# jim-ec/constraint_solver

Measured on AMD Instinct MI355X. Metric: body·substeps/sec at 262k rigid bodies, 20 substeps/frame; 1/2/4/8 GPU, higher is better.
Workload: dtype f64

## Files before the change

constraint_solver_amd/csrc/xpbd_pairs.h:

```cpp
#pragma once

#include <cstdint>
#include <hip/hip_runtime_api.h>

#include "xpbd_kernels.h"

namespace xpbd {

struct ShapeDesc {
    uint32_t vert0, n_verts;
    uint32_t face0, n_faces;
    uint32_t edge0, n_edges;
    uint32_t dir0, n_dirs;
};

struct PolytopeTables {
    const double *verts;
    const double *planes;
    const double *centroids;
    const ShapeDesc *desc;
    const uint32_t *face_start;
    const uint32_t *face_verts;
    const uint32_t *edges;
    const double *radii;
    const double *edge_dirs;
    const uint32_t *edge_dir_id;
    uint32_t n_shapes;
    uint32_t total_verts;
    uint32_t max_verts, max_faces, max_face_verts;
    const uint8_t *shape_class;
    uint32_t two_classes;
    uint32_t small_max_face_verts;
};

constexpr uint32_t kMaxManifoldPoints = 8;
constexpr uint32_t kMaxFaceVerts = 8;
constexpr double kEdgeBias = 1e-6;

struct Manifold {
    uint32_t n_points;
    uint32_t feature;
    uint32_t index_a, index_b;
    double separation;
    double p_ref[kMaxManifoldPoints][3];
    double p_inc[kMaxManifoldPoints][3];
};

struct alignas(256) ContactManifold {
    double plane[4];
    double point[kMaxManifoldPoints][3];
};
static_assert(sizeof(ContactManifold) == 256, "plane + four points = the first 128-byte line");
constexpr uint32_t kPairCodeFeatureShift = 4;
constexpr uint32_t kSurvivorCounters = 4;

struct EdgeQuery {
    double separation;
    uint32_t edge_a, edge_b;
};
hipError_t launch_edge_axes_reference(const BodyArrays &b, const PolytopeTables &t, const double *frames, const uint32_t *pairs,
                                      uint32_t n_pairs, EdgeQuery *out, hipStream_t stream);


struct SatScratch {
    uint32_t *counters;
    uint32_t *survivors;
    uint32_t calls;
    uint16_t *axis_cache;
    bool cache_edge_axes;
};

hipError_t launch_sat_pairs(const BodyArrays &b, const PolytopeTables &t, const double *frames, const uint32_t *pairs,
                            uint32_t n_pairs, Manifold *out, hipStream_t stream);
hipError_t launch_pair_pretest(const BodyArrays &b, const PolytopeTables &t, const double *frames, const uint32_t *pairs,
                               uint32_t n_pairs, uint8_t *codes, SatScratch &list, uint32_t **count, uint32_t **next_count,
                               hipStream_t stream, bool use_axis_cache = false, const double *gjk_axis_cache = nullptr);
hipError_t launch_sat_contacts(const BodyArrays &b, const PolytopeTables &t, const double *frames, const uint32_t *pairs,
                               uint32_t n_pairs, ContactManifold *out, uint8_t *codes, SatScratch *list,
                               hipStream_t stream, bool dense = false);

}
```

constraint_solver_amd/csrc/xpbd_pairs.hip:

```cpp
#include <cfloat>
#include <cstdlib>

#include <type_traits>

#include "xpbd_clip.hpp"
#include "xpbd_device.hpp"
#include "xpbd_pairs.h"

namespace xpbd {
namespace {

constexpr uint32_t kMaxV = XPBD_MAX_SHAPE_VERTS;
#ifndef XPBD_SAT_MIN_WAVES_PER_SIMD
#define XPBD_SAT_MIN_WAVES_PER_SIMD 4
#endif
#ifndef XPBD_SAT_BOX_LANES
#define XPBD_SAT_BOX_LANES 8
#endif
#ifndef XPBD_SAT_DENSE_BOX_LANES
#define XPBD_SAT_DENSE_BOX_LANES 4
#endif
#ifndef XPBD_SAT_SMALL_LANES
#define XPBD_SAT_SMALL_LANES 16
#endif
#ifndef XPBD_SAT_LS_LANES
#define XPBD_SAT_LS_LANES 16
#endif
#ifndef XPBD_SAT_MID_LANES
#define XPBD_SAT_MID_LANES 32
#endif
#ifndef XPBD_SAT_TIMING_STOP
#define XPBD_SAT_TIMING_STOP 0
#endif
#ifndef XPBD_SAT_EDGE_CACHE_GAP
#define XPBD_SAT_EDGE_CACHE_GAP 1.0e-5
#endif
constexpr uint32_t kNone = 0xFFFFFFFFu;
constexpr uint32_t kAxisCacheEdge = 0x8000u;
constexpr uint32_t kWidePairCount = 32768;

template <uint32_t V, uint32_t P, uint32_t PW>
struct PairLds {
    static constexpr uint32_t kVerts = V;
    static_assert(kMaxFaceVerts <= V, "the reference face reuses vertex rows");
    static constexpr uint32_t kScratchRows = P > V ? P : V;
    static constexpr uint32_t kBaseDwords = 2 * (2 * V * 3 + 2 * kScratchRows * 3);
    static constexpr uint32_t pad_dwords()
    {
        if (PW == 1)
            return 0;
        uint32_t best = 64;
        for (uint32_t odd = 1; odd < 2 * PW; odd += 2) {
            const uint32_t pad = (odd * (64 / PW) + 64 - kBaseDwords % 64) % 64;
            best = pad < best ? pad : best;
        }
        return best;
    }
    static constexpr uint32_t kPadDwords = pad_dwords();
    double world[2][V][3];
    union {
        double local[2][V][3];
        double poly[2][P][3];
    };
    uint32_t pad[kPadDwords ? kPadDwords : 2];
};

__device__ __forceinline__ bool finite3(Vec3 v)
{
    return fabs(v.x) <= DBL_MAX && fabs(v.y) <= DBL_MAX && fabs(v.z) <= DBL_MAX;
}

__device__ __forceinline__ Vec3 support_last_max(const double (*verts)[3], uint32_t n, Vec3 dir)
{
    Vec3 best = ld3(verts, 0);
    long long best_key = total_key(dot(best, dir));
    for (uint32_t k = 1; k < n; ++k) {
        const Vec3 x = ld3(verts, k);
        const long long key = total_key(dot(x, dir));
        if (best_key <= key) {
            best_key = key;
            best = x;
        }
    }
    return best;
}

__device__ __forceinline__ double clamp01(double x) { return x < 0.0 ? 0.0 : (x > 1.0 ? 1.0 : x); }

template <uint32_t L, class Lds, class M>
__device__ __forceinline__ void sat_pair(Lds &s, const BodyArrays &b, const PolytopeTables &t, const double *__restrict__ frames,
                                         const uint32_t *__restrict__ pairs, uint32_t p, M *__restrict__ out, uint32_t lane,
                                         uint16_t *__restrict__ axis_cache = nullptr, uint8_t *__restrict__ codes = nullptr, bool cache_edge_axes = false)
{
    constexpr uint32_t H = L / 2;
    constexpr uint32_t P = (Lds::kVerts <= 8 && L <= 8) ? 8 : 16;
    const uint32_t ia = pairs[2 * (size_t)p], ib = pairs[2 * (size_t)p + 1];
    const Frame fa = load_record_p1(frames, ia), fb = load_record_p1(frames, ib);
    const Frame fa_inv = inverse(fa), fb_inv = inverse(fb);
    const uint32_t sa = b.shape_id[ia], sb = b.shape_id[ib];
    const ShapeDesc da = t.desc[sa], db = t.desc[sb];

    M *m = out + p;
    auto answer = [&](uint32_t n_points, uint32_t feature, uint32_t index_a, uint32_t index_b, double separation) {
        if (codes)
            codes[p] = (uint8_t)(n_points | (feature << kPairCodeFeatureShift));
        set_header(*m, n_points, feature, index_a, index_b, separation);
    };
    auto no_contact = [&]() {
        if (codes)
            codes[p] = 0;
        else
            set_header(*m, 0, 0, 0, 0, 0.0);
    };
    if (da.n_verts == 0 || db.n_verts == 0 || da.n_faces == 0 || db.n_faces == 0) {
        if (lane == 0)
            no_contact();
        return;
    }

    const uint32_t half = lane / H, k = lane % H;
    {
        const ShapeDesc dm = half ? db : da;
        for (uint32_t vtx = k; vtx < dm.n_verts; vtx += H) {
            const double *v = t.verts + 3 * (size_t)(dm.vert0 + vtx);
            const Vec3 w = (half ? fb : fa) * Vec3{v[0], v[1], v[2]};
            st3(s.world[half], vtx, w);
            st3(s.local[half], vtx, (half ? fa_inv : fb_inv) * w);
        }
    }
    __syncthreads();

    double fdist = -DBL_MAX;
    uint32_t fidx = kNone;
    {
        const ShapeDesc dm = half ? db : da;
        const uint32_t n_other = half ? da.n_verts : db.n_verts;
        for (uint32_t f = k; f < dm.n_faces; f += H) {
            const double *pl = t.planes + 4 * (size_t)(dm.face0 + f);
            const Vec3 n{pl[0], pl[1], pl[2]};
            const Vec3 sup = support_last_max(s.local[half ^ 1u], n_other, -n);
            const double dist = dot(n, sup) - pl[3];
            if (dist > fdist) {
                fdist = dist;
                fidx = f;
            }
        }
    }
    reduce_max_first(fdist, fidx, H);
    const double fdist_other = partner(fdist, H);
    const uint32_t fidx_other = partner(fidx, H);
    const double qa = half ? fdist_other : fdist, qb = half ? fdist : fdist_other;
    const uint32_t face_a = half ? fidx_other : fidx, face_b = half ? fidx : fidx_other;
    if (qa >= 0.0 || qb >= 0.0 || face_a == kNone || face_b == kNone) {
        if (lane == 0) {
            no_contact();
            if (axis_cache)
                axis_cache[p] = (uint16_t)(qa >= 0.0 ? 1u + 2u * face_a : (qb >= 0.0 ? 2u + 2u * face_b : 0u));
        }
        return;
    }
    if (axis_cache && lane == 0)
        axis_cache[p] = 0;
#if XPBD_SAT_TIMING_STOP == 1
    if (lane == 0)
        no_contact();
    return;
#endif

    double ebest = -DBL_MAX;
    uint32_t eq = kNone;
    const double *cca = t.centroids + 3 * (size_t)sa, *ccb = t.centroids + 3 * (size_t)sb;
    const Vec3 a_to_b = fb * Vec3{ccb[0], ccb[1], ccb[2]} - fa * Vec3{cca[0], cca[1], cca[2]};
    const bool dirs_staged = da.n_dirs <= Lds::kVerts && db.n_dirs <= Lds::kVerts;
    __syncthreads();
    if (dirs_staged) {
        for (uint32_t d = lane; d < da.n_dirs + db.n_dirs; d += L) {
            const bool of_b = d >= da.n_dirs;
            const uint32_t kd = of_b ? d - da.n_dirs : d;
            const double *dd = t.edge_dirs + 3 * (size_t)((of_b ? db.dir0 : da.dir0) + kd);
            st3(s.local[of_b ? 1 : 0], kd, (of_b ? fb : fa).rotation * Vec3{dd[0], dd[1], dd[2]});
        }
        __syncthreads();
    }
    auto edge_axis = [&](uint32_t i, uint32_t j, Vec3 &axis) -> bool {
        Vec3 n;
        if (dirs_staged) {
            n = normalized(cross(ld3(s.local[0], i), ld3(s.local[1], j)));
        } else {
            const double *da_ = t.edge_dirs + 3 * (size_t)(da.dir0 + i), *db_ = t.edge_dirs + 3 * (size_t)(db.dir0 + j);
            n = normalized(cross(fa.rotation * Vec3{da_[0], da_[1], da_[2]}, fb.rotation * Vec3{db_[0], db_[1], db_[2]}));
        }
        if (!finite3(n))
            return false;
        if (dot(n, a_to_b) < 0.0)
            n = -n;
        axis = n;
        return true;
    };
    {
        const uint32_t total = da.n_dirs * db.n_dirs;
        for (uint32_t q = lane; q < total; q += L) {
            const uint32_t i = q / db.n_dirs, j = q - i * db.n_dirs;
            Vec3 axis;
            if (!edge_axis(i, j, axis))
                continue;
            double reach_a = dot(ld3(s.world[0], 0), axis), reach_b = dot(ld3(s.world[1], 0), axis);
            for (uint32_t v = 1; v < da.n_verts; ++v) {
                const double rr = dot(ld3(s.world[0], v), axis);
                if (rr > reach_a)
                    reach_a = rr;
            }
            for (uint32_t v = 1; v < db.n_verts; ++v) {
                const double rr = dot(ld3(s.world[1], v), axis);
                if (rr < reach_b)
                    reach_b = rr;
            }
            const double dist = reach_b - reach_a;
            if (dist > ebest) {
                ebest = dist;
                eq = q;
            }
        }
    }
    reduce_max_first(ebest, eq, L);
    if (ebest >= 0.0) {
        if (lane == 0) {
            no_contact();
            if (axis_cache && cache_edge_axes && ebest > XPBD_SAT_EDGE_CACHE_GAP)
                axis_cache[p] = (uint16_t)(kAxisCacheEdge | eq);
        }
        return;
    }

#if XPBD_SAT_TIMING_STOP == 2
    if (lane == 0)
        no_contact();
    return;
#endif
    const double face_best = qa > qb ? qa : qb;
    const bool use_edges = eq != kNone && ebest > face_best + kEdgeBias;

    if (use_edges) {
        const uint32_t di = eq / db.n_dirs, dj = eq - di * db.n_dirs;
        Vec3 axis;
        (void)edge_axis(di, dj, axis);
        double sa_best = -DBL_MAX, sb_best = DBL_MAX;
        uint32_t edge_i = kNone, edge_j = kNone;
        for (uint32_t e = lane; e < da.n_edges; e += L) {
            if (t.edge_dir_id[da.edge0 + e] != di)
                continue;
            const uint32_t *ev = t.edges + 2 * (size_t)(da.edge0 + e);
            const double sp = dot(ld3(s.world[0], ev[0]), axis) + dot(ld3(s.world[0], ev[1]), axis);
            if (sp > sa_best) {
                sa_best = sp;
                edge_i = e;
            }
        }
        for (uint32_t e = lane; e < db.n_edges; e += L) {
            if (t.edge_dir_id[db.edge0 + e] != dj)
                continue;
            const uint32_t *ev = t.edges + 2 * (size_t)(db.edge0 + e);
            const double sp = dot(ld3(s.world[1], ev[0]), axis) + dot(ld3(s.world[1], ev[1]), axis);
            if (sp < sb_best) {
                sb_best = sp;
                edge_j = e;
            }
        }
        reduce_max_first(sa_best, edge_i, L);
        reduce_min_first(sb_best, edge_j, L);
        if (edge_i == kNone)
            edge_i = 0;
        if (edge_j == kNone)
            edge_j = 0;
        if (lane == 0) {
            const uint32_t i = edge_i, j = edge_j;
            const uint32_t *ea = t.edges + 2 * (size_t)(da.edge0 + i), *eb = t.edges + 2 * (size_t)(db.edge0 + j);
            const Vec3 a0 = ld3(s.world[0], ea[0]), a1 = ld3(s.world[0], ea[1]);
            const Vec3 b0 = ld3(s.world[1], eb[0]), b1 = ld3(s.world[1], eb[1]);
            const Vec3 d1 = a1 - a0, d2 = b1 - b0, r = a0 - b0;
            const double a = dot(d1, d1), e = dot(d2, d2), f = dot(d2, r), c = dot(d1, r), bb = dot(d1, d2);
            const double denom = a * e - bb * bb;
            double sp = clamp01((bb * f - c * e) / denom);
            double tp = (bb * sp + f) / e;
            if (tp < 0.0) {
                tp = 0.0;
                sp = clamp01(-c / a);
            } else if (tp > 1.0) {
                tp = 1.0;
                sp = clamp01((bb - c) / a);
            }
            const Vec3 pa = a0 + d1 * sp, pb = b0 + d2 * tp;
            answer(1, 2, i, j, ebest);
            set_single_contact(*m, pb, pa);
        }
        return;
    }

    const uint32_t r = (qa == face_best) ? 0u : 1u;
    const uint32_t ref_face = r ? face_b : face_a;
    const Frame fr = r ? fb : fa, fi = r ? fa : fb;
    const ShapeDesc dr = r ? db : da, di = r ? da : db;
    uint32_t iface;
    const uint32_t n_out = face_contact_group<L, P>(t, dr, di, fr, fi, ref_face, s.world[r], s.world[r ^ 1u], s.poly[0], s.poly[1],
                                                    s.world[r ^ 1u], m, lane, iface);
    if (lane != 0)
        return;
    answer(n_out, r, r ? iface : face_a, r ? face_b : iface, face_best);
}

__device__ __forceinline__ bool tight_spheres_overlap(const BodyArrays &b, const PolytopeTables &t, const double *__restrict__ frames,
                                                      const uint32_t *__restrict__ pairs, uint32_t p)
{
    const uint32_t ia = pairs[2 * (size_t)p], ib = pairs[2 * (size_t)p + 1];
    const uint32_t sa = b.shape_id[ia], sb = b.shape_id[ib];
    const double *ca = t.centroids + 3 * (size_t)sa, *cb = t.centroids + 3 * (size_t)sb;
    const Vec3 between = load_record_p1(frames, ib) * Vec3{cb[0], cb[1], cb[2]} - load_record_p1(frames, ia) * Vec3{ca[0], ca[1], ca[2]};
    const double reach = t.radii[sa] + t.radii[sb];
    return dot(between, between) < reach * reach;
}

template <uint32_t L, uint32_t V>
struct SatLds {
    static constexpr uint32_t PW = 64 / L;
    static constexpr uint32_t P = (V <= 8 && L <= 8) ? 8 : 16;
    static_assert(V == 8 || V == 16 || V == kMaxV, "vertex capacity per body");
    using Record = PairLds<V, P, PW>;
    static_assert(sizeof(Record) % 8 == 0, "pair records must stay 8-byte aligned");
};

template <uint32_t L, uint32_t V, bool PRETEST, class M>
__global__ void __launch_bounds__(64, XPBD_SAT_MIN_WAVES_PER_SIMD) k_sat_pairs(BodyArrays b, PolytopeTables t,
                                                                               const double *__restrict__ frames,
                                                                               const uint32_t *__restrict__ pairs, uint32_t n_pairs,
                                                                               M *__restrict__ out, uint8_t *__restrict__ codes)
{
    using Lds = typename SatLds<L, V>::Record;
    __shared__ Lds s_all[SatLds<L, V>::PW];
    const uint32_t group = threadIdx.x / L, lane = threadIdx.x % L;
    const uint32_t p = blockIdx.x * SatLds<L, V>::PW + group;
    if (p >= n_pairs)
        return;
    if (PRETEST && !tight_spheres_overlap(b, t, frames, pairs, p)) {
        if (lane == 0)
            codes[p] = 0;
        return;
    }
    sat_pair<L>(s_all[group], b, t, frames, pairs, p, out, lane, nullptr, codes);
}

constexpr uint32_t kPretestBlock = 1024;

__device__ __forceinline__ bool cached_direction_separates(const BodyArrays &b, const PolytopeTables &t, const double *__restrict__ frames,
                                                           const uint32_t *__restrict__ pairs, uint32_t p, Vec3 d)
{
    const uint32_t ia = pairs[2 * (size_t)p], ib = pairs[2 * (size_t)p + 1];
    const Frame fa = load_record_p1(frames, ia), fb = load_record_p1(frames, ib);
    const ShapeDesc da = t.desc[b.shape_id[ia]], db = t.desc[b.shape_id[ib]];
    if (da.n_verts == 0 || db.n_verts == 0)
        return false;
    auto support = [&](const ShapeDesc &ds, Vec3 dir) {
        Vec3 best{0.0, 0.0, 0.0};
        long long best_key = 0;
        for (uint32_t k = 0; k < ds.n_verts; ++k) {
            const double *v = t.verts + 3 * (size_t)(ds.vert0 + k);
            const Vec3 x{v[0], v[1], v[2]};
            const long long key = total_key(dot(x, dir));
            if (k == 0 || best_key <= key) {
                best_key = key;
                best = x;
            }
        }
        return best;
    };
    const Vec3 a = fa * support(da, conjugate(fa.rotation) * d), bb = fb * support(db, conjugate(fb.rotation) * (-d));
    return !(dot(a - bb, d) > 0.0);
}

__device__ __forceinline__ bool cached_face_separates(const BodyArrays &b, const PolytopeTables &t, const double *__restrict__ frames,
                                                      const uint32_t *__restrict__ pairs, uint32_t p, uint32_t code)
{
    const uint32_t owner = (code - 1u) & 1u, face = (code - 1u) >> 1;
    const uint32_t ia = pairs[2 * (size_t)p], ib = pairs[2 * (size_t)p + 1];
    const Frame fa = load_record_p1(frames, ia), fb = load_record_p1(frames, ib);
    const ShapeDesc da = t.desc[b.shape_id[ia]], db = t.desc[b.shape_id[ib]];
    const ShapeDesc dx = owner ? db : da, dy = owner ? da : db;
    if (face >= dx.n_faces || dy.n_verts == 0)
        return false;
    const Frame fy = owner ? fa : fb, fx_inv = inverse(owner ? fb : fa);
    const double *pl = t.planes + 4 * (size_t)(dx.face0 + face);
    const Vec3 n{pl[0], pl[1], pl[2]}, dir = -n;
    Vec3 best{0.0, 0.0, 0.0};
    long long best_key = 0;
    for (uint32_t k = 0; k < dy.n_verts; ++k) {
        const double *v = t.verts + 3 * (size_t)(dy.vert0 + k);
        const Vec3 w = fy * Vec3{v[0], v[1], v[2]};
        const Vec3 local = fx_inv * w;
        const long long key = total_key(dot(local, dir));
        if (k == 0 || best_key <= key) {
            best_key = key;
            best = local;
        }
    }
    return dot(n, best) - pl[3] >= 0.0;
}

__device__ __forceinline__ bool cached_edge_axis_separates(const BodyArrays &b, const PolytopeTables &t, const double *__restrict__ frames,
                                                           const uint32_t *__restrict__ pairs, uint32_t p, uint32_t q)
{
    const uint32_t ia = pairs[2 * (size_t)p], ib = pairs[2 * (size_t)p + 1];
    const Frame fa = load_record_p1(frames, ia), fb = load_record_p1(frames, ib);
    const uint32_t sa = b.shape_id[ia], sb = b.shape_id[ib];
    const ShapeDesc da = t.desc[sa], db = t.desc[sb];
    if (da.n_verts == 0 || db.n_verts == 0 || db.n_dirs == 0)
        return false;
    const uint32_t i = q / db.n_dirs, j = q - i * db.n_dirs;
    if (i >= da.n_dirs)
        return false;
    const double *da_ = t.edge_dirs + 3 * (size_t)(da.dir0 + i), *db_ = t.edge_dirs + 3 * (size_t)(db.dir0 + j);
    Vec3 n = normalized(cross(fa.rotation * Vec3{da_[0], da_[1], da_[2]}, fb.rotation * Vec3{db_[0], db_[1], db_[2]}));
    if (!finite3(n))
        return false;
    const double *cca = t.centroids + 3 * (size_t)sa, *ccb = t.centroids + 3 * (size_t)sb;
    const Vec3 a_to_b = fb * Vec3{ccb[0], ccb[1], ccb[2]} - fa * Vec3{cca[0], cca[1], cca[2]};
    if (dot(n, a_to_b) < 0.0)
        n = -n;
    double reach_a = 0.0, reach_b = 0.0;
    for (uint32_t v = 0; v < da.n_verts; ++v) {
        const double *x = t.verts + 3 * (size_t)(da.vert0 + v);
        const double rr = dot(fa * Vec3{x[0], x[1], x[2]}, n);
        if (v == 0 || rr > reach_a)
            reach_a = rr;
    }
    for (uint32_t v = 0; v < db.n_verts; ++v) {
        const double *x = t.verts + 3 * (size_t)(db.vert0 + v);
        const double rr = dot(fb * Vec3{x[0], x[1], x[2]}, n);
        if (v == 0 || rr < reach_b)
            reach_b = rr;
    }
    return reach_b - reach_a >= 0.0;
}

template <bool CLASSES>
__global__ void __launch_bounds__(kPretestBlock) k_pair_pretest(BodyArrays b, PolytopeTables t, const double *__restrict__ frames,
                                                                const uint32_t *__restrict__ pairs, uint32_t n_pairs,
                                                                uint8_t *__restrict__ codes, uint32_t *__restrict__ survivor_count,
                                                                uint32_t *__restrict__ survivors, const uint16_t *__restrict__ axis_cache,
                                                                const double *__restrict__ gjk_axis_cache)
{
    constexpr uint32_t NC = CLASSES ? 3 : 1;
    constexpr uint32_t NP = 3, NW = kPretestBlock / 64;
    __shared__ uint32_t wave_base[NC][NP][NW];
    __shared__ uint32_t list_base[NC];
    const uint32_t p = blockIdx.x * kPretestBlock + threadIdx.x, lane = threadIdx.x & 63u, wave = threadIdx.x >> 6;
    bool keep = false;
    uint32_t cls = 0, path = 0;
    if (p < n_pairs) {
        const uint32_t last = codes[p];
        path = last == 0 ? 0u : ((last >> kPairCodeFeatureShift) == 2u ? 2u : 1u);
        keep = tight_spheres_overlap(b, t, frames, pairs, p);
        if (keep && axis_cache) {
            const uint32_t code = axis_cache[p];
            if (code & kAxisCacheEdge ? cached_edge_axis_separates(b, t, frames, pairs, p, code & (kAxisCacheEdge - 1u))
                                      : (code && cached_face_separates(b, t, frames, pairs, p, code)))
                keep = false;
        }
        if (keep && gjk_axis_cache) {
            const double *c = gjk_axis_cache + 3 * (size_t)p;
            const Vec3 d{c[0], c[1], c[2]};
            if (dot(d, d) > 0.0 && cached_direction_separates(b, t, frames, pairs, p, d))
                keep = false;
        }
        if (!keep)
            codes[p] = 0;
        else if (CLASSES) {
            const uint32_t ca = t.shape_class[b.shape_id[pairs[2 * (size_t)p]]], cb = t.shape_class[b.shape_id[pairs[2 * (size_t)p + 1]]];
            cls = ca + cb;
        }
    }
    unsigned long long mine = 0;
#pragma unroll
    for (uint32_t c = 0; c < NC; ++c)
#pragma unroll
        for (uint32_t q = 0; q < NP; ++q) {
            const unsigned long long mask = __ballot(keep && cls == c && path == q);
            if (lane == 0)
                wave_base[c][q][wave] = (uint32_t)__popcll(mask);
            if (cls == c && path == q)
                mine = mask;
        }
    __syncthreads();
    if (threadIdx.x < NC) {
        const uint32_t c = threadIdx.x;
        uint32_t run = 0;
        for (uint32_t q = 0; q < NP; ++q)
            for (uint32_t w = 0; w < NW; ++w) {
                const uint32_t n = wave_base[c][q][w];
                wave_base[c][q][w] = run;
                run += n;
            }
        list_base[c] = run ? atomicAdd(survivor_count + c, run) : 0u;
    }
    __syncthreads();
    if (keep) {
        const uint32_t at = list_base[cls] + wave_base[cls][path][wave] + (uint32_t)__popcll(mine & ((1ull << lane) - 1ull));
        survivors[cls == 0 ? at : (cls == 1 ? n_pairs - 1u - at : n_pairs + at)] = p;
    }
}

template <uint32_t L, uint32_t V>
__global__ void __launch_bounds__(64, XPBD_SAT_MIN_WAVES_PER_SIMD) k_sat_survivors(BodyArrays b, PolytopeTables t,
                                                                                   const double *__restrict__ frames,
                                                                                   const uint32_t *__restrict__ pairs,
                                                                                   const uint32_t *__restrict__ survivor_count,
                                                                                   uint32_t *__restrict__ next_survivor_counts,
                                                                                   const uint32_t *__restrict__ survivors, uint32_t back_n,
                                                                                   ContactManifold *__restrict__ out, uint16_t *__restrict__ axis_cache,
                                                                                   uint8_t *__restrict__ codes, bool cache_edge_axes)
{
    using Lds = typename SatLds<L, V>::Record;
    __shared__ Lds s_all[SatLds<L, V>::PW];
    const uint32_t group = threadIdx.x / L, lane = threadIdx.x % L;
    const uint32_t k = blockIdx.x * SatLds<L, V>::PW + group;
    const uint32_t n = *survivor_count;
    if (blockIdx.x == 0 && threadIdx.x < kSurvivorCounters)
        next_survivor_counts[threadIdx.x] = 0;
    if (k >= n)
        return;
    sat_pair<L>(s_all[group], b, t, frames, pairs, survivors[back_n ? back_n - 1u - k : k], out, lane, axis_cache, codes, cache_edge_axes);
}

struct EdgeLds {
    double world[2][kMaxV][3];
};

__device__ __forceinline__ Vec3 support_last_max_position(const double (*verts)[3], uint32_t n, Vec3 dir)
{
    return support_last_max(verts, n, dir);
}

__global__ void __launch_bounds__(64) k_edge_axes_reference(BodyArrays b, PolytopeTables t, const double *__restrict__ frames,
                                                            const uint32_t *__restrict__ pairs, uint32_t n_pairs, EdgeQuery *__restrict__ out)
{
    __shared__ EdgeLds s;
    const uint32_t p = blockIdx.x, lane = threadIdx.x;
    if (p >= n_pairs)
        return;
    const uint32_t ia = pairs[2 * (size_t)p], ib = pairs[2 * (size_t)p + 1];
    const Frame fa = load_record_p1(frames, ia), fb = load_record_p1(frames, ib);
    const uint32_t sa = b.shape_id[ia], sb = b.shape_id[ib];
    const ShapeDesc da = t.desc[sa], db = t.desc[sb];
    for (uint32_t v = lane; v < da.n_verts + db.n_verts; v += 64) {
        const bool of_b = v >= da.n_verts;
        const uint32_t k = of_b ? v - da.n_verts : v;
        const double *x = t.verts + 3 * (size_t)((of_b ? db.vert0 : da.vert0) + k);
        st3(s.world[of_b ? 1 : 0], k, (of_b ? fb : fa) * Vec3{x[0], x[1], x[2]});
    }
    __syncthreads();
    const double *cca = t.centroids + 3 * (size_t)sa;
    const Vec3 centroid_a = fa * Vec3{cca[0], cca[1], cca[2]};
    double best = -DBL_MAX;
    uint32_t best_q = kNone;
    const uint32_t total = da.n_edges * db.n_edges;
    for (uint32_t q = lane; q < total; q += 64) {
        const uint32_t ie = q / db.n_edges, je = q - ie * db.n_edges;
        const uint32_t *ea = t.edges + 2 * (size_t)(da.edge0 + ie), *eb = t.edges + 2 * (size_t)(db.edge0 + je);
        const Vec3 foot = ld3(s.world[0], ea[0]);
        const Vec3 e0 = ld3(s.world[0], ea[1]) - foot;
        const Vec3 e1 = ld3(s.world[1], eb[1]) - ld3(s.world[1], eb[0]);
        Vec3 axis = normalized(cross(e0, e1));
        if (dot(axis, foot - centroid_a) < 0.0)
            axis = -axis;
        if (da.n_verts == 0 || db.n_verts == 0)
            continue;
        if (dot(support_last_max_position(s.world[0], da.n_verts, axis), axis) > dot(foot, axis))
            continue;
        const Plane plane = plane_from_point_normal(foot, axis);
        const double dist = distance(plane, support_last_max_position(s.world[1], db.n_verts, -axis));
        if (dist > best) {
            best = dist;
            best_q = q;
        }
    }
    reduce_max_first(best, best_q, 64);
    if (lane == 0) {
        out[p].separation = best;
        out[p].edge_a = best_q == kNone ? kNone : best_q / db.n_edges;
        out[p].edge_b = best_q == kNone ? kNone : best_q % db.n_edges;
    }
}

}

namespace {
uint32_t wide_pair_count()
{
    const char *e = std::getenv("XPBD_SAT_WIDE_PAIRS");
    return e ? (uint32_t)std::strtoul(e, nullptr, 10) : kWidePairCount;
}

template <class Launch>
void for_shape_maxima(uint32_t max_verts, uint32_t max_faces, uint32_t max_face_verts, uint32_t n_pairs, bool dense, Launch launch)
{
    const uint32_t wide = wide_pair_count();
    if (max_verts <= 8 && max_faces <= 8 && max_face_verts <= 4 && dense && n_pairs >= 2 * (size_t)wide)
        launch(std::integral_constant<uint32_t, XPBD_SAT_DENSE_BOX_LANES>{}, std::integral_constant<uint32_t, 8>{});
    else if (max_verts <= 8 && max_faces <= 8 && max_face_verts <= 4 && n_pairs >= wide)
        launch(std::integral_constant<uint32_t, XPBD_SAT_BOX_LANES>{}, std::integral_constant<uint32_t, 8>{});
    else if (max_verts <= 8 && max_faces <= 8)
        launch(std::integral_constant<uint32_t, XPBD_SAT_SMALL_LANES>{}, std::integral_constant<uint32_t, 8>{});
    else if (max_verts <= 16)
        launch(std::integral_constant<uint32_t, XPBD_SAT_MID_LANES>{}, std::integral_constant<uint32_t, 16>{});
    else
        launch(std::integral_constant<uint32_t, 64>{}, std::integral_constant<uint32_t, kMaxV>{});
}

template <class Launch>
void for_shape_class(const PolytopeTables &t, uint32_t n_pairs, bool dense, Launch launch)
{
    for_shape_maxima(t.max_verts, t.max_faces, t.max_face_verts, n_pairs, dense, launch);
}
}

hipError_t launch_sat_pairs(const BodyArrays &b, const PolytopeTables &t, const double *frames, const uint32_t *pairs,
                            uint32_t n_pairs, Manifold *out, hipStream_t stream)
{
    if (n_pairs)
        for_shape_class(t, n_pairs, false, [&](auto lanes, auto verts) {
            constexpr uint32_t L = decltype(lanes)::value, V = decltype(verts)::value;
            hipLaunchKernelGGL((k_sat_pairs<L, V, false, Manifold>), dim3((n_pairs + 64 / L - 1) / (64 / L)), dim3(64), 0, stream, b, t,
                               frames, pairs, n_pairs, out, nullptr);
        });
    return hipGetLastError();
}

hipError_t launch_edge_axes_reference(const BodyArrays &b, const PolytopeTables &t, const double *frames, const uint32_t *pairs,
                                      uint32_t n_pairs, EdgeQuery *out, hipStream_t stream)
{
    if (n_pairs)
        hipLaunchKernelGGL(k_edge_axes_reference, dim3(n_pairs), dim3(64), 0, stream, b, t, frames, pairs, n_pairs, out);
    return hipGetLastError();
}

hipError_t launch_pair_pretest(const BodyArrays &b, const PolytopeTables &t, const double *frames, const uint32_t *pairs,
                               uint32_t n_pairs, uint8_t *codes, SatScratch &list, uint32_t **count, uint32_t **next_count,
                               hipStream_t stream, bool use_axis_cache, const double *gjk_axis_cache)
{
    *count = list.counters + kSurvivorCounters * (list.calls & 1u);
    *next_count = list.counters + kSurvivorCounters * ((list.calls + 1u) & 1u);
    ++list.calls;
    hipLaunchKernelGGL(k_pair_pretest<false>, dim3((n_pairs + kPretestBlock - 1) / kPretestBlock), dim3(kPretestBlock), 0, stream, b, t, frames,
                       pairs, n_pairs, codes, *count, list.survivors, use_axis_cache ? list.axis_cache : nullptr, gjk_axis_cache);
    return hipGetLastError();
}

hipError_t launch_sat_contacts(const BodyArrays &b, const PolytopeTables &t, const double *frames, const uint32_t *pairs,
                               uint32_t n_pairs, ContactManifold *out, uint8_t *codes, SatScratch *list, hipStream_t stream, bool dense)
{
    if (n_pairs == 0)
        return hipSuccess;
    if (list && t.two_classes) {
        uint32_t *count = list->counters + kSurvivorCounters * (list->calls & 1u);
        uint32_t *next = list->counters + kSurvivorCounters * ((list->calls + 1u) & 1u);
        ++list->calls;
        hipLaunchKernelGGL(k_pair_pretest<true>, dim3((n_pairs + kPretestBlock - 1) / kPretestBlock), dim3(kPretestBlock), 0, stream, b, t,
                           frames, pairs, n_pairs, codes, count, list->survivors, list->axis_cache, nullptr);
        for_shape_maxima(8, 8, t.small_max_face_verts, n_pairs, dense, [&](auto lanes, auto verts) {
            constexpr uint32_t L = decltype(lanes)::value, V = decltype(verts)::value;
            hipLaunchKernelGGL((k_sat_survivors<L, V>), dim3((n_pairs + 64 / L - 1) / (64 / L)), dim3(64), 0, stream, b, t, frames, pairs, count,
                               next, list->survivors, 0u, out, list->axis_cache, codes, list->cache_edge_axes);
        });
        if (t.max_verts <= 16)
            hipLaunchKernelGGL((k_sat_survivors<XPBD_SAT_LS_LANES, 16>), dim3((n_pairs + 64 / XPBD_SAT_LS_LANES - 1) / (64 / XPBD_SAT_LS_LANES)), dim3(64), 0,
                               stream, b, t, frames, pairs, count + 1, next, list->survivors, n_pairs, out, list->axis_cache, codes, list->cache_edge_axes);
        else
            hipLaunchKernelGGL((k_sat_survivors<32, kMaxV>), dim3((n_pairs + 1) / 2), dim3(64), 0, stream, b, t, frames, pairs, count + 1, next,
                               list->survivors, n_pairs, out, list->axis_cache, codes, list->cache_edge_axes);
        for_shape_class(t, n_pairs, dense, [&](auto lanes, auto verts) {
            constexpr uint32_t L = decltype(lanes)::value, V = decltype(verts)::value;
            hipLaunchKernelGGL((k_sat_survivors<L, V>), dim3((n_pairs + 64 / L - 1) / (64 / L)), dim3(64), 0, stream, b, t, frames, pairs,
                               count + 2, next, list->survivors + n_pairs, 0u, out, list->axis_cache, codes, list->cache_edge_axes);
        });
        return hipGetLastError();
    }
    for_shape_class(t, n_pairs, dense, [&](auto lanes, auto verts) {
        constexpr uint32_t L = decltype(lanes)::value, V = decltype(verts)::value;
        const dim3 grid((n_pairs + 64 / L - 1) / (64 / L));
        if (list) {
            uint32_t *count = nullptr, *next = nullptr;
            (void)launch_pair_pretest(b, t, frames, pairs, n_pairs, codes, *list, &count, &next, stream, true);
            hipLaunchKernelGGL((k_sat_survivors<L, V>), grid, dim3(64), 0, stream, b, t, frames, pairs, count, next, list->survivors, 0u, out,
                               list->axis_cache, codes, list->cache_edge_axes);
        } else {
            hipLaunchKernelGGL((k_sat_pairs<L, V, true, ContactManifold>), grid, dim3(64), 0, stream, b, t, frames, pairs, n_pairs, out, codes);
        }
    });
    return hipGetLastError();
}

}
```

constraint_solver_amd/csrc/xpbd_world.hpp:

```cpp
#pragma once

#include <cstdint>
#include <limits>
#include <utility>
#include <vector>

#include <hip/hip_runtime_api.h>

#include "xpbd_internal.h"
#include "xpbd_kernels.h"
#include "xpbd_contacts.h"
#include "xpbd_gjk.h"
#include "xpbd_islands.h"
#include "xpbd_joint_state.h"
#include "xpbd_kinematic.h"
#include "xpbd_pairs.h"
#include "xpbd_population_remap.hpp"
#include "xpbd_query.h"
#include "xpbd_report.h"
#include "xpbd_sleep.h"

struct xpbd_world;

#pragma GCC visibility push(hidden)

using xpbd::DeviceBuffer;
using xpbd::set_error;

constexpr uint32_t kMaxBodies = 0xFFFFFF00u;
template <class T> constexpr T at_least_one(T n) { return n ? n : 1; }
inline uint32_t stride_for(uint32_t n_bodies) { return (at_least_one(n_bodies) + 255u) / 256u * 256u; }
inline uint32_t next_pow2(uint32_t v)
{
    uint32_t p = 1;
    while (p < v)
        p <<= 1;
    return p;
}

struct JointTables {
    xpbd::JointSet set;
    std::vector<xpbd_joint_limit> slide_limits;
    struct Csr {
        uint32_t n = 0;
        DeviceBuffer joints, off, list;
    } csr;
    struct Limits {
        uint32_t n_limits = 0;
        DeviceBuffer limits, limit_off;
    } limits;
    struct Extras {
        uint32_t n_extra_joints = 0;
        DeviceBuffer sums, joints, slots, off, items;
        DeviceBuffer joint_slot, drive_item;
        std::vector<uint32_t> drive_item_host;
        bool targets_on_device = false;
    } extras;

    void fill(xpbd::ContactBuffers &c) const
    {
        c.joints = csr.joints.as<xpbd::Joint>();
        c.joint_off = csr.off.as<uint32_t>();
        c.joint_list = csr.list.as<uint32_t>();
        c.limits = limits.limits.as<xpbd::JointLimit>();
        c.limit_off = limits.limit_off.as<uint32_t>();
        c.joint_extra = extras.sums.as<double>();
        c.extra_joints = extras.joints.as<uint32_t>();
        c.extra_slots = extras.slots.as<uint32_t>();
        c.extra_off = extras.off.as<uint32_t>();
        c.extra_items = extras.items.as<xpbd::JointExtraItem>();
        c.n_extra_joints = extras.n_extra_joints;
    }
    xpbd::JointStateTables state_tables() const
    {
        return xpbd::JointStateTables{csr.joints.as<xpbd::Joint>(), csr.n, limits.limits.as<xpbd::JointLimit>(), limits.limit_off.as<uint32_t>(),
                                      extras.joint_slot.as<uint32_t>(), extras.off.as<uint32_t>(), extras.items.as<xpbd::JointExtraItem>()};
    }
    xpbd::DriveTable drive_table() const
    {
        return xpbd::DriveTable{extras.items.as<xpbd::JointExtraItem>(), extras.drive_item.as<uint32_t>(), (uint32_t)extras.drive_item_host.size()};
    }
    void clear() { *this = JointTables{}; }
};

struct KinematicBodies {
    std::vector<xpbd_kinematic> list;
    DeviceBuffer table;
    bool targets_on_device = false;

    bool any() const { return !list.empty(); }
    xpbd::KinematicTable view() const { return xpbd::KinematicTable{table.as<xpbd_kinematic>(), (uint32_t)list.size()}; }
    void clear() { *this = KinematicBodies{}; }
};

struct Broadphase {
    DeviceBuffer centers, radius, cell, key, maxr, grid_partials, bucket_start, bucket_cursor, items, items_unsorted, slot_sphere,
        slot_cell, slot_filter, slot_inert, nbr_off, pair_first, upper_start, nbr, nbr_pair, pairs, manifolds, pair_codes, scan;
    uint32_t table_size = 0, n_entries = 0, n_pairs = 0;
    bool have_neighbours = false;
    struct Totals {
        uint32_t entries, pairs;
        unsigned long long stats[2];
    };
    Totals *totals = nullptr;
    hipEvent_t event = nullptr;
    bool pending = false;

    Broadphase() = default;
    Broadphase(const Broadphase &) = delete;
    Broadphase &operator=(const Broadphase &) = delete;
    ~Broadphase() { release_host(); }
    void release_host() noexcept
    {
        if (totals)
            (void)hipHostFree(totals);
        if (event)
            (void)hipEventDestroy(event);
        totals = nullptr;
        event = nullptr;
    }
    void fill(xpbd::ContactBuffers &c) const
    {
        c.centers = centers.as<double>();
        c.radius = radius.as<double>();
        c.cell = cell.as<int32_t>();
        c.key = key.as<uint32_t>();
        c.grid = maxr.as<xpbd::GridInfo>();
        c.grid_partials = grid_partials.as<double>();
        c.bucket_start = bucket_start.as<uint32_t>();
        c.bucket_cursor = bucket_cursor.as<uint32_t>();
        c.items = items.as<uint32_t>();
        c.items_unsorted = items_unsorted.as<uint32_t>();
        c.table_size = table_size;
        c.slot_sphere = slot_sphere.as<double>();
        c.slot_cell = slot_cell.as<int32_t>();
        c.nbr_off = nbr_off.as<uint32_t>();
        c.pair_first = pair_first.as<uint32_t>();
        c.upper_start = upper_start.as<uint32_t>();
        c.nbr = nbr.as<uint32_t>();
        c.nbr_pair = nbr_pair.as<uint32_t>();
        c.pairs = pairs.as<uint32_t>();
        c.manifolds = manifolds.as<xpbd::ContactManifold>();
        c.pair_codes = pair_codes.as<uint8_t>();
        c.scan_scratch = scan.as<uint32_t>();
    }
};

struct NarrowphaseSchedule {
    DeviceBuffer stats;
    DeviceBuffer sat_counters, sat_survivors, sat_axis_cache, gjk_axis_cache;
    xpbd::SatScratch sat_scratch{nullptr, nullptr, 0, nullptr, true};
    bool sat_two_pass = false;
    uint32_t sat_schedule = XPBD_SAT_SCHEDULE_AUTO;
    unsigned long long stats_touching_seen = 0, stats_pair_substeps = 0, stats_pair_substeps_seen = 0;
    DeviceBuffer gjk_counters, gjk_pairs_scratch;
    xpbd::GjkScratch gjk_scratch{nullptr, nullptr, 0, nullptr, nullptr};

    void choose(unsigned long long touching_now, uint32_t two_classes);
    int ensure_gjk_scratch(uint32_t n_pairs, hipStream_t stream);
};

struct ContactReport {
    bool on = false;
    bool frame = false;
    bool keys_ready = false;
    bool ready = false;
    bool prev_valid = false;
    uint32_t substeps = 0, cur = 0;
    uint32_t counts[4] = {0, 0, 0, 0};
    uint32_t *host = nullptr;
    DeviceBuffer touch, flag, sel, npts, keys[2], scan, ev_flag, pairs, points, events;
    const uint8_t *map_owned = nullptr;
    const uint32_t *map_ids = nullptr;

    ContactReport() = default;
    ContactReport(const ContactReport &) = delete;
    ContactReport &operator=(const ContactReport &) = delete;
    ~ContactReport() { release_host(); }
    void release_host() noexcept
    {
        if (host)
            (void)hipHostFree(host);
        host = nullptr;
    }

    void reset()
    {
        frame = keys_ready = ready = prev_valid = false;
        substeps = 0;
    }
    void release_buffers()
    {
        for (DeviceBuffer *b : {&touch, &flag, &sel, &npts, &keys[0], &keys[1], &scan, &ev_flag, &pairs, &points, &events})
            b->release();
    }
    xpbd::ReportFrame frame_of(const Broadphase &bp) const
    {
        return xpbd::ReportFrame{bp.pairs.as<uint32_t>(), bp.pair_codes.as<uint8_t>(), bp.manifolds.as<xpbd::ContactManifold>(),
                                 touch.as<uint32_t>(), bp.n_pairs, map_owned, map_ids};
    }
    int compact_keys(const xpbd_world *w);
    int frame_end(const xpbd_world *w);
    int frame_begin(const xpbd_world *w);
    int note_substep(const xpbd_world *w, const uint8_t *pair_codes);
    int prepare(const xpbd_world *w, const char *who);

    struct ShardLoan {
        ContactReport &r;
        ShardLoan(ContactReport &report, const uint8_t *owned, const uint32_t *ids) : r(report)
        {
            r.map_owned = owned;
            r.map_ids = ids;
            r.keys_ready = r.ready = false;
        }
        ~ShardLoan()
        {
            r.map_owned = nullptr;
            r.map_ids = nullptr;
            r.keys_ready = r.ready = false;
        }
    };
};

struct ReplanStaging {
    DeviceBuffer aos, shape, src, incoming, keys, records;
};
struct FrameSnapshot {
    DeviceBuffer state;
    bool valid = false, stepped = false;
};
struct TerrainStaging {
    DeviceBuffer xy, out;
};
struct EditStaging {
    DeviceBuffer indices, values, list;
    DeviceBuffer owner;
};
struct PopulationScratch {
    DeviceBuffer remove, indices, prefix, scan, map, src;
};
struct History {
    DeviceBuffer states;
    uint32_t length = 0;
    std::vector<uint8_t> stepped;
    std::vector<uint8_t> sleep_requests;
};

struct Islands {
    DeviceBuffer parent, fixed, flag, scan, result, island_of, records;

    int reserve(const xpbd_world *w, bool host_island_of, uint32_t host_records);
    int enqueue(xpbd_world *w, uint32_t flags, uint32_t *dev_island_of, xpbd_island *dev_records, uint32_t cap, uint32_t *dev_total);
};

struct Sleep {
    bool on = false, fresh = true;
    bool moving = false;
    xpbd_sleep_config cfg{};
    uint32_t requests = 0;
    DeviceBuffer state, scratch;

    static size_t state_bytes(uint32_t stride) { return (size_t)stride * 13 + xpbd::kSleepCtrlWords * 4; }
    xpbd::SleepState view(const xpbd_world *w) const;
    const uint8_t *asleep(const xpbd_world *w) const { return view(w).asleep; }
    void wake_all(bool zero_counters)
    {
        if (on)
            requests |= xpbd::kSleepWakeAll | (zero_counters ? xpbd::kSleepZeroCounters : 0u);
    }
    int ensure(const xpbd_world *w);
    int frame_begin(xpbd_world *w);
    int frame_records(xpbd_world *w, uint32_t *trace, uint32_t trace_rows);
    int frame_end(xpbd_world *w);
    int request(xpbd_world *w, const uint32_t *dev_indices, uint32_t every, uint32_t n);
    int request_drives(xpbd_world *w, const uint32_t *dev_drives, const double *dev_targets, uint32_t n);
};

#pragma GCC visibility pop

struct xpbd_world {
    int device = 0;
    uint32_t mode = XPBD_MODE_FUSED;
    uint32_t flags = 0;
    uint32_t block_size = 0;

    hipStream_t own_stream = nullptr;
    hipStream_t stream = nullptr;

    uint32_t n = 0;
    uint32_t stride = 0;
    uint32_t max_shape_id = 0;
    DeviceBuffer dyn, stat, shape_id, aos_staging, last_mask, trace, block_counts, contacts;
    uint32_t trace_rows = 0;
    bool stepped = false;

    DeviceBuffer shape_verts, shape_offsets;
    uint32_t n_shapes = 0, total_verts = 0;

    DeviceBuffer planes, centroids, shape_desc, face_start, face_verts, edges, pair_buf, manifold_buf;
    DeviceBuffer shape_radii, edge_dirs, edge_dir_id, shape_class;
    uint32_t two_classes = 0, small_max_face_verts = 0;
    bool has_topology = false;
    uint32_t max_verts = 0, max_faces = 0, max_face_verts = 0;
    xpbd::PolytopeTables tables() const
    {
        return xpbd::PolytopeTables{shape_verts.as<double>(), planes.as<double>(), centroids.as<double>(),
                                    shape_desc.as<xpbd::ShapeDesc>(), face_start.as<uint32_t>(),
                                    face_verts.as<uint32_t>(), edges.as<uint32_t>(), shape_radii.as<double>(),
                                    edge_dirs.as<double>(), edge_dir_id.as<uint32_t>(), n_shapes, total_verts, max_verts, max_faces, max_face_verts,
                                    shape_class.as<uint8_t>(), two_classes, small_max_face_verts};
    }

    double contact_pad = 0.02;
    double max_depenetration_speed = 0.0;
    uint32_t narrowphase = XPBD_NARROWPHASE_SAT;
    DeviceBuffer dyn_alt, cb_rec, cb_rec_b, cb_stat_rec, cb_stat_shape;
    bool stat_rec_valid = false;
    bool stat_shared = false;
    std::vector<double> stat_shape_host;
    std::vector<uint8_t> stat_shape_seen;
    Broadphase bp;
    NarrowphaseSchedule np;
    ContactReport report;
    ReplanStaging replan;
    FrameSnapshot snapshot;
    JointTables joints;
    struct Filters {
        bool on = false;
        uint32_t flags = 0;
        void clear() { *this = Filters{}; }
    } filters;
    DeviceBuffer ft_filters;
    struct Materials {
        bool on = false;
        double ground_friction = std::numeric_limits<double>::infinity();
        void clear() { *this = Materials{}; }
    } materials;
    DeviceBuffer mt_friction;
    struct Restitution {
        bool on = false;
        double ground = 0.0, bounce_threshold = 0.0;
        void clear() { *this = Restitution{}; }
    } restitution;
    DeviceBuffer rs_restitution, rs_start;
    KinematicBodies kinematics;
    xpbd::Terrain terrain{};
    DeviceBuffer tr_planes;
    DeviceBuffer tr_heights;
    TerrainStaging terrain_staging;
    xpbd::SceneQueryScratch query;
    EditStaging edit;
    PopulationScratch pop;
    History history;
    Islands islands;
    Sleep sleep;
    size_t history_slot_bytes() const
    {
        return ((size_t)xpbd::kDynFields * stride * 8 + (size_t)stride * 4 + (sleep.on ? Sleep::state_bytes(stride) : 0) + 255) / 256 * 256;
    }

    xpbd::ContactBuffers contact_buffers(uint32_t frame_set = 0) const
    {
        xpbd::ContactBuffers c{};
        bp.fill(c);
        c.rec = (frame_set ? cb_rec_b : cb_rec).as<double>();
        c.stat_rec = stat_shared ? cb_stat_shape.as<double>() : cb_stat_rec.as<double>();
        c.stat_index = stat_shared ? shape_id.as<uint32_t>() : nullptr;
        c.stats = np.stats.as<unsigned long long>();
        joints.fill(c);
        c.filter = filters.on ? ft_filters.as<uint2>() : nullptr;
        c.slot_filter = filters.on ? bp.slot_filter.as<uint32_t>() : nullptr;
        c.filter_jointed = (filters.flags & XPBD_FILTER_JOINTED) ? 1u : 0u;
        c.max_depenetration_speed = max_depenetration_speed;
        c.friction = materials.on ? mt_friction.as<double>() : nullptr;
        c.ground_friction = materials.ground_friction;
        c.restitution = restitution.on ? rs_restitution.as<double>() : nullptr;
        c.ground_restitution = restitution.ground;
        c.bounce_threshold = restitution.bounce_threshold;
        c.terrain = terrain;
        return c;
    }

    xpbd::InertBodies inert_bodies() const
    {
        return sleep.on ? xpbd::InertBodies{sleep.view(this).inert, bp.slot_inert.as<uint8_t>()} : xpbd::InertBodies{};
    }

    xpbd::BodyArrays arrays() const
    {
        return xpbd::BodyArrays{dyn.as<double>(), stat.as<double>(), shape_id.as<uint32_t>(), stride, n};
    }
    xpbd::ShapeTable shapes() const
    {
        return xpbd::ShapeTable{shape_verts.as<double>(), shape_offsets.as<uint32_t>(), n_shapes, total_verts};
    }

    ~xpbd_world()
    {
        (void)hipSetDevice(device);
        if (stream)
            (void)hipStreamSynchronize(stream);
        bp.release_host();
        report.release_host();
        if (own_stream)
            (void)hipStreamDestroy(own_stream);
    }
};

#pragma GCC visibility push(hidden)

inline xpbd::SleepState Sleep::view(const xpbd_world *w) const
{
    const size_t st = w->stride;
    xpbd::SleepState s{};
    s.rest_frames = state.as<uint32_t>();
    s.group = s.rest_frames + st;
    s.mark = s.group + st;
    s.ctrl = s.mark + st;
    s.asleep = reinterpret_cast<uint8_t *>(s.ctrl + xpbd::kSleepCtrlWords);
    s.island_min = scratch.as<uint32_t>();
    s.fixed = reinterpret_cast<uint8_t *>(s.island_min + st);
    s.inert = s.fixed + st;
    s.moving = s.inert + st;
    s.n = w->n;
    s.stride = w->stride;
    return s;
}

inline int bind_device(const xpbd_world *w)
{
    XPBD_HIP_TRY(hipSetDevice(w->device));
    return XPBD_OK;
}

void absorb_stat_record(xpbd_world *w, const xpbd_rigid &body, uint32_t sid);
void reset_stat_records(xpbd_world *w, bool start_over, uint32_t n);
void take_body_count(xpbd_world *w, uint32_t n_new, uint32_t max_shape_id);
void drop_body_settings(xpbd_world *w);
int adopt_body_count(xpbd_world *w, uint32_t n_new, uint32_t max_shape_id);
int stage_upload(DeviceBuffer &fresh, const void *values, size_t bytes);
int upload_table(DeviceBuffer &table, const void *values, size_t bytes);
int stage_joint_tables(xpbd::JointSet set, uint32_t n_bodies, hipStream_t stream, JointTables &out);

int sync_drive_targets(xpbd_world *w);

int sync_kinematic_targets(xpbd_world *w);

int build_neighbours_enqueue(xpbd_world *w, double dt);
int build_neighbours_collect(xpbd_world *w);
int build_neighbours(xpbd_world *w, double dt);
int narrowphase_contacts(xpbd_world *w, const xpbd::BodyArrays &b, const xpbd::ContactBuffers &c);
int substep_contacts(xpbd_world *w, double h, uint32_t *trace, uint32_t trace_row, const xpbd::BodySubset &awake = xpbd::BodySubset(),
                     uint32_t kinematic_left = 0);
int step_contacts(xpbd_world *w, double dt, double h, uint32_t substeps, uint32_t *trace);

#pragma GCC visibility pop
```

Before: 16.95 billion.

## Merge three SAT survivor-class launches into one persistent grid-stride kernel

Replaces the three per-class survivor SAT launches (small-small, large-small, large-large) with a single persistent kernel that walks each class's survivor list in grid-stride loops, sharing one LDS union. The grid is sized from the occupancy API (CUs times blocks per CU times a rounds factor) and cached per kernel form. The aim is to cut launch overhead and the oversized grids that were sized to n_pairs rather than the actual survivor counts, letting classes backfill each other. In exchange the LDS footprint is the maximum of the three layouts, the combined kernel may use more registers, and a __syncthreads per iteration adds some overhead. It is on by default and can be disabled via an environment variable.

```diff
diff --git a/constraint_solver_amd/csrc/xpbd_pairs.h b/constraint_solver_amd/csrc/xpbd_pairs.h
--- a/constraint_solver_amd/csrc/xpbd_pairs.h
+++ b/constraint_solver_amd/csrc/xpbd_pairs.h
@@ -62,12 +62,19 @@
                                       uint32_t n_pairs, EdgeQuery *out, hipStream_t stream);
 
 
+struct SatGrids {
+    static constexpr uint32_t kForms = 4;
+    const void *form[kForms];
+    uint32_t blocks[kForms];
+    uint32_t next;
+};
 struct SatScratch {
     uint32_t *counters;
     uint32_t *survivors;
     uint32_t calls;
     uint16_t *axis_cache;
     bool cache_edge_axes;
+    SatGrids grids;
 };
 
 hipError_t launch_sat_pairs(const BodyArrays &b, const PolytopeTables &t, const double *frames, const uint32_t *pairs,
diff --git a/constraint_solver_amd/csrc/xpbd_pairs.hip b/constraint_solver_amd/csrc/xpbd_pairs.hip
--- a/constraint_solver_amd/csrc/xpbd_pairs.hip
+++ b/constraint_solver_amd/csrc/xpbd_pairs.hip
@@ -529,6 +529,54 @@
     sat_pair<L>(s_all[group], b, t, frames, pairs, survivors[back_n ? back_n - 1u - k : k], out, lane, axis_cache, codes, cache_edge_axes);
 }
 
+struct SatSurvivorArgs {
+    const double *frames;
+    const uint32_t *pairs;
+    ContactManifold *out;
+    uint16_t *axis_cache;
+    uint8_t *codes;
+    bool cache_edge_axes;
+};
+
+template <uint32_t L, uint32_t V>
+__device__ __forceinline__ void sat_survivor_walk(typename SatLds<L, V>::Record *s_all, const BodyArrays &b, const PolytopeTables &t,
+                                                  const SatSurvivorArgs &a, uint32_t n, const uint32_t *__restrict__ survivors, uint32_t back_n)
+{
+    constexpr uint32_t PW = SatLds<L, V>::PW;
+    const uint32_t stride = gridDim.x * PW;
+    for (uint32_t base = blockIdx.x * PW; base < n; base += stride) {
+        uint32_t thread = threadIdx.x;
+        asm volatile("" : "+v"(thread));
+        const uint32_t group = thread / L, lane = thread % L;
+        const uint32_t k = base + group;
+        if (k < n)
+            sat_pair<L>(s_all[group], b, t, a.frames, a.pairs, survivors[back_n ? back_n - 1u - k : k], a.out, lane, a.axis_cache, a.codes,
+                        a.cache_edge_axes);
+        __syncthreads();
+        if (n - base <= stride)
+            break;
+    }
+}
+
+template <uint32_t L0, uint32_t V0, uint32_t L1, uint32_t V1, uint32_t L2, uint32_t V2>
+__global__ void __launch_bounds__(64, XPBD_SAT_MIN_WAVES_PER_SIMD) k_sat_survivors_all(BodyArrays b, PolytopeTables t, SatSurvivorArgs a,
+                                                                                       const uint32_t *__restrict__ survivor_counts,
+                                                                                       uint32_t *__restrict__ next_survivor_counts,
+                                                                                       const uint32_t *__restrict__ survivors, uint32_t n_pairs)
+{
+    __shared__ union {
+        typename SatLds<L0, V0>::Record small_small[SatLds<L0, V0>::PW];
+        typename SatLds<L1, V1>::Record large_small[SatLds<L1, V1>::PW];
+        typename SatLds<L2, V2>::Record large_large[SatLds<L2, V2>::PW];
+    } s;
+    const uint32_t n0 = survivor_counts[0], n1 = survivor_counts[1], n2 = survivor_counts[2];
+    if (blockIdx.x == 0 && threadIdx.x < kSurvivorCounters)
+        next_survivor_counts[threadIdx.x] = 0;
+    sat_survivor_walk<L2, V2>(s.large_large, b, t, a, n2, survivors + n_pairs, 0u);
+    sat_survivor_walk<L1, V1>(s.large_small, b, t, a, n1, survivors, n_pairs);
+    sat_survivor_walk<L0, V0>(s.small_small, b, t, a, n0, survivors, 0u);
+}
+
 struct EdgeLds {
     double world[2][kMaxV][3];
 };
@@ -619,6 +667,60 @@
 {
     for_shape_maxima(t.max_verts, t.max_faces, t.max_face_verts, n_pairs, dense, launch);
 }
+
+bool sat_merged()
+{
+    const char *e = std::getenv("XPBD_SAT_MERGED");
+    return !e || std::strtoul(e, nullptr, 10) != 0;
+}
+
+#ifndef XPBD_SAT_GRID_ROUNDS
+#define XPBD_SAT_GRID_ROUNDS 8
+#endif
+constexpr uint32_t kMaxPersistentWaves = 1u << 20;
+template <class Kernel>
+hipError_t persistent_waves(Kernel kernel, SatGrids &grids, uint32_t *blocks)
+{
+    if (const char *e = std::getenv("XPBD_SAT_PERSISTENT_WAVES")) {
+        const unsigned long v = std::strtoul(e, nullptr, 10);
+        if (v) {
+            *blocks = v < kMaxPersistentWaves ? (uint32_t)v : kMaxPersistentWaves;
+            return hipSuccess;
+        }
+    }
+    const void *form = reinterpret_cast<const void *>(kernel);
+    for (uint32_t i = 0; i < SatGrids::kForms; ++i)
+        if (grids.form[i] == form) {
+            *blocks = grids.blocks[i];
+            return hipSuccess;
+        }
+    int device = 0, cus = 0, per_cu = 0;
+    hipError_t e = hipGetDevice(&device);
+    if (e == hipSuccess)
+        e = hipDeviceGetAttribute(&cus, hipDeviceAttributeMultiprocessorCount, device);
+    if (e == hipSuccess)
+        e = hipOccupancyMaxActiveBlocksPerMultiprocessor(&per_cu, kernel, 64, 0);
+    if (e != hipSuccess)
+        return e;
+    if (cus < 1 || per_cu < 1)
+        return hipErrorInvalidValue;
+    const uint32_t slot = grids.next++ % SatGrids::kForms;
+    grids.form[slot] = form;
+    *blocks = grids.blocks[slot] = (uint32_t)cus * (uint32_t)per_cu * XPBD_SAT_GRID_ROUNDS;
+    return hipSuccess;
+}
+
+template <uint32_t L0, uint32_t V0, uint32_t L1, uint32_t V1, uint32_t L2, uint32_t V2>
+hipError_t launch_sat_survivors_all(const BodyArrays &b, const PolytopeTables &t, const SatSurvivorArgs &a, const uint32_t *count, uint32_t *next,
+                                    SatScratch &list, uint32_t n_pairs, hipStream_t stream)
+{
+    uint32_t blocks = 0;
+    const hipError_t e = persistent_waves(k_sat_survivors_all<L0, V0, L1, V1, L2, V2>, list.grids, &blocks);
+    if (e != hipSuccess)
+        return e;
+    hipLaunchKernelGGL((k_sat_survivors_all<L0, V0, L1, V1, L2, V2>), dim3(blocks), dim3(64), 0, stream, b, t, a, count, next, list.survivors, n_pairs);
+    return hipGetLastError();
+}
 }
 
 hipError_t launch_sat_pairs(const BodyArrays &b, const PolytopeTables &t, const double *frames, const uint32_t *pairs,
@@ -664,6 +766,23 @@
         ++list->calls;
         hipLaunchKernelGGL(k_pair_pretest<true>, dim3((n_pairs + kPretestBlock - 1) / kPretestBlock), dim3(kPretestBlock), 0, stream, b, t,
                            frames, pairs, n_pairs, codes, count, list->survivors, list->axis_cache, nullptr);
+        if (sat_merged()) {
+            const SatSurvivorArgs a{frames, pairs, out, list->axis_cache, codes, list->cache_edge_axes};
+            hipError_t status = hipSuccess;
+            for_shape_maxima(8, 8, t.small_max_face_verts, n_pairs, dense, [&](auto lanes0, auto verts0) {
+                for_shape_class(t, n_pairs, dense, [&](auto lanes2, auto verts2) {
+                    constexpr uint32_t L0 = decltype(lanes0)::value, V0 = decltype(verts0)::value;
+                    constexpr uint32_t L2 = decltype(lanes2)::value, V2 = decltype(verts2)::value;
+                    if constexpr (V0 == 8 && V2 == 16)
+                        status = launch_sat_survivors_all<L0, V0, XPBD_SAT_LS_LANES, 16, L2, V2>(b, t, a, count, next, *list, n_pairs, stream);
+                    else if constexpr (V0 == 8 && V2 == kMaxV)
+                        status = launch_sat_survivors_all<L0, V0, 32, kMaxV, L2, V2>(b, t, a, count, next, *list, n_pairs, stream);
+                    else
+                        status = hipErrorInvalidValue;
+                });
+            });
+            return status;
+        }
         for_shape_maxima(8, 8, t.small_max_face_verts, n_pairs, dense, [&](auto lanes, auto verts) {
             constexpr uint32_t L = decltype(lanes)::value, V = decltype(verts)::value;
             hipLaunchKernelGGL((k_sat_survivors<L, V>), dim3((n_pairs + 64 / L - 1) / (64 / L)), dim3(64), 0, stream, b, t, frames, pairs, count,
diff --git a/constraint_solver_amd/csrc/xpbd_world.hpp b/constraint_solver_amd/csrc/xpbd_world.hpp
--- a/constraint_solver_amd/csrc/xpbd_world.hpp
+++ b/constraint_solver_amd/csrc/xpbd_world.hpp
@@ -149,7 +149,7 @@
 struct NarrowphaseSchedule {
     DeviceBuffer stats;
     DeviceBuffer sat_counters, sat_survivors, sat_axis_cache, gjk_axis_cache;
-    xpbd::SatScratch sat_scratch{nullptr, nullptr, 0, nullptr, true};
+    xpbd::SatScratch sat_scratch{nullptr, nullptr, 0, nullptr, true, {}};
     bool sat_two_pass = false;
     uint32_t sat_schedule = XPBD_SAT_SCHEDULE_AUTO;
     unsigned long long stats_touching_seen = 0, stats_pair_substeps = 0, stats_pair_substeps_seen = 0;
```

Result: no change. 16.98 billion (median of 3 runs) (+0.2%).
